# sakehl/SKA-SDP-Accelerate-gridding

Measured on AMD Instinct MI355X. Metric: Mvis/s gridded (w-proj, 4096^2 grid), higher is better.
Workload: dtype f64

## Files before the change

ska-sdp-accelerate-gridding_amd/csrc/tile_sorted.hip:

```cpp
#include "tile_common.h"

namespace gridhip {

__device__ __forceinline__ double readlane_f64(double x, int l)
{
    return __hiloint2double(__builtin_amdgcn_readlane(__double2hiint(x), l),
                            __builtin_amdgcn_readlane(__double2loint(x), l));
}

constexpr int SORTED_IM_OFF = 65528;

__device__ const int cut15[3][16] = {{0, 106, 211, 317, 422, 500, 578, 655, 733, 781, 829, 877, 926, 958, 991, 1024},
                                     {0, 108, 221, 329, 434, 513, 596, 677, 754, 800, 852, 898, 943, 969, 998, 1024},
                                     {0, 100, 202, 303, 401, 480, 562, 641, 718, 769, 824, 875, 925, 957, 992, 1024}};

struct SortedItem {
    int32_t valid, tile, grp, staged;
};

template <int S, bool DEGRID, int ABL = 0, bool AW = false, bool BT = false>
__global__ void __launch_bounds__(1024, 4) tile_grid_sorted_kernel(Geom g, const RecWord *__restrict__ recs,
                                                                const int32_t *__restrict__ bin_start,
                                                                const int32_t *__restrict__ work_start,
                                                                const double2 *__restrict__ gcf,
                                                                double2 *__restrict__ vis,
                                                                double *__restrict__ grid, int nkeys, int batch,
                                                                int32_t *__restrict__ scalars,
                                                                double2 *__restrict__ sorted_vals,
                                                                uint2 *__restrict__ sorted_mo)
{
    extern __shared__ double lds[];
    constexpr int S2 = S * S;
    constexpr int TAIL0 = S2 - ((S2 + 63) / 64 - 1) * 64;
    constexpr int EXTRA = DEGRID ? 0 : (TAIL0 > 32 && TAIL0 <= 34) ? TAIL0 - 32 : (S2 > 256 && TAIL0 <= 2) ? TAIL0 : 0;
    constexpr int S2E = S2 - EXTRA;
    constexpr int NSTEP_ALL = (S2E + 63) / 64;
    constexpr int TAIL = S2E - (NSTEP_ALL - 1) * 64;
    constexpr int MAXST = DEGRID ? 4 : 5;
    constexpr int FP = (NSTEP_ALL + MAXST - 1) / MAXST;
    constexpr int KST = (NSTEP_ALL + FP - 1) / FP;
    constexpr int REM = NSTEP_ALL % FP;
    constexpr int PBASE = NSTEP_ALL / FP;
    constexpr int NSTEP = KST;
    constexpr int LASTS = (REM == 0 ? KST : KST - 1) - 1;
    constexpr bool PAIR = !DEGRID && TAIL == 32;
    const int tid = threadIdx.x, nthr = blockDim.x;
    const int lane = tid & 63, wave = __builtin_amdgcn_readfirstlane(tid >> 6), nw = nthr >> 6;
    const int plane = g.lrows * g.ldw;
    const int IMO = BT ? g.imoff / 8 : SORTED_IM_OFF / 8;
    double *lre = lds, *lim = lds + IMO;
    int32_t *hist = reinterpret_cast<int32_t *>(lim + plane);
    const int hist_words = (nkeys + 1 + 3) & ~3;
    SortedItem *desc = reinterpret_cast<SortedItem *>(hist + hist_words);
    double2 *svals_wg = sorted_vals + (size_t)blockIdx.x * 2 * batch;
    uint2 *smo_wg = sorted_mo + (size_t)blockIdx.x * 2 * batch;
    int32_t *sorig_wg = reinterpret_cast<int32_t *>(sorted_vals) + (size_t)blockIdx.x * 2 * batch;

    constexpr bool STAGE_VALS = !DEGRID && AW;
    constexpr bool STAGE_ORIG = DEGRID && AW;
    const bool solo = nw == 1;
    const bool is_sorter = wave == nw - 1;
    if (is_sorter && !solo && !(g.dbg & 512)) __builtin_amdgcn_s_setprio(3);
    const bool is_walker = solo || !is_sorter;
    const int nwalk = solo ? 1 : nw - 1;
    const int ncell = g.lrows * g.lcols;

    if (blockIdx.x == 0 && tid == 0) {
        long long *st = reinterpret_cast<long long *>(scalars + 20);
        st[0] = (long long)__builtin_amdgcn_s_memtime();
        st[1] = (long long)__builtin_amdgcn_s_memrealtime();
    }
    long long prof[7] = {0, 0, 0, 0, 0, 0, 0}, pt = 0;
#define GH_STAMP(i_)                        \
    if ((ABL & 16) && lane == 0) {          \
        const long long now_ = clock64();   \
        prof[i_] += now_ - pt;              \
        pt = now_;                          \
    }
    if ((ABL & 16) && lane == 0) pt = clock64();

    int32_t *queue = scalars + 4;
    int turn = 0;
    int items_left = ((int)blockIdx.x >= g.npersist) ? g.budget : 0x7fffffff;
    auto prepare = [&](int slot) {
        WorkItem w;
        int grp = 0;
        bool have = false;
        if (items_left <= 0) turn = g.ngroups;
        --items_left;
        while (turn < g.ngroups) {
            grp = (blockIdx.x + turn) % g.ngroups;
            int item = 0;
            if (lane == 0) item = atomicAdd(&queue[grp], 1);
            item = __builtin_amdgcn_readfirstlane(item);
            if (find_work_at(g, bin_start, work_start, grp, item, &w)) {
                have = true;
                break;
            }
            ++turn;
        }
        if (!have) {
            if (lane == 0) desc[slot].valid = 0;
            return;
        }
        GH_STAMP(0)
        const int first_plane = (grp * g.W + g.ngroups - 1) / g.ngroups;
        const int first_slice = first_plane * g.Q * g.Q * g.P;
        double2 *svals = svals_wg + (size_t)slot * batch;
        uint2 *smo = smo_wg + (size_t)slot * batch;
        int32_t *sorig = sorig_wg + (size_t)slot * batch;
        const int b_lo = w.v_lo;
        const int cnt = min(batch, w.v_hi - b_lo);
        for (int i = lane; i <= nkeys; i += 64) hist[i] = 0;
        __builtin_amdgcn_fence(__ATOMIC_ACQ_REL, "wavefront");
        __builtin_amdgcn_wave_barrier();
        for (int r0 = lane; r0 < cnt; r0 += 8 * 64) {
            int key[8];
#pragma unroll
            for (int q = 0; q < 8; ++q) {
                bool off;
                key[q] = load_rec(recs, b_lo + min(r0 + q * 64, cnt - 1), g, &off).kslice - first_slice;
                if (AW) key[q] = (int)((unsigned)key[q] % (unsigned)nkeys);
                if (off) key[q] = -1;
            }
#pragma unroll
            for (int q = 0; q < 8; ++q)
                if (r0 + q * 64 < cnt && (unsigned)key[q] < (unsigned)nkeys) atomicAdd(&hist[key[q]], 1);
        }
        __builtin_amdgcn_fence(__ATOMIC_ACQ_REL, "wavefront");
        __builtin_amdgcn_wave_barrier();
        GH_STAMP(1)
        {
            const int per = (nkeys + 63) / 64;
            const int lo = min(lane * per, nkeys), hi = min(lo + per, nkeys);
            int sum = 0;
            for (int i = lo; i < hi; ++i) sum += hist[i];
            int incl = sum;
#pragma unroll
            for (int off = 1; off < 64; off <<= 1) {
                const int t = __shfl_up(incl, off, 64);
                if (lane >= off) incl += t;
            }
            int base = incl - sum;
            for (int i = lo; i < hi; ++i) {
                const int c = hist[i];
                hist[i] = base;
                base += c;
            }
        }
        __builtin_amdgcn_fence(__ATOMIC_ACQ_REL, "wavefront");
        __builtin_amdgcn_wave_barrier();
        GH_STAMP(2)
        int bad = 0;
        for (int r0 = lane; r0 < cnt; r0 += 8 * 64) {
            VisRec rec[8];
            double2 val[8];
            bool off[8];
#pragma unroll
            for (int q = 0; q < 8; ++q) rec[q] = load_rec(recs, b_lo + min(r0 + q * 64, cnt - 1), g, &off[q]);
            if (STAGE_VALS) {
#pragma unroll
                for (int q = 0; q < 8; ++q) val[q] = (ABL & 8) ? make_double2(1.0, (double)q) : load_nt(vis + rec[q].orig);
            }
#pragma unroll
            for (int q = 0; q < 8; ++q) {
                if (r0 + q * 64 >= cnt) break;
                int key = rec[q].kslice - first_slice;
                if (AW) key = (int)((unsigned)key % (unsigned)nkeys);
                if (off[q] || (unsigned)key >= (unsigned)nkeys) {
                    ++bad;
                    continue;
                }
                const int pos = atomicAdd(&hist[key], 1);
                if ((unsigned)pos < (unsigned)batch) {
                    smo[pos] = make_uint2(((uint32_t)key << 16) | (uint32_t)((rec[q].lxy >> 16) * g.ldw + (rec[q].lxy & 0xffff)),
                                          (uint32_t)(AW ? rec[q].kslice : rec[q].orig));
                    if (STAGE_VALS) svals[pos] = val[q];
                    if (STAGE_ORIG) sorig[pos] = rec[q].orig;
                } else
                    ++bad;
            }
        }
        if (bad) atomicAdd(&scalars[2], bad);
        __builtin_amdgcn_fence(__ATOMIC_ACQ_REL, "wavefront");
        __builtin_amdgcn_wave_barrier();
        if (lane == 0) {
            SortedItem d;
            d.valid = 1;
            d.tile = w.tile;
            d.grp = grp;
            d.staged = hist[nkeys - 1];
            desc[slot] = d;
        }
        GH_STAMP(3)
    };

    int loff[NSTEP];
    const bool tail_ok = lane < TAIL || TAIL == 64;
#pragma unroll
    for (int s = 0; s < NSTEP; ++s) {
        int t = s * 64 + lane;
        if (FP == 1 && s == NSTEP - 1 && !tail_ok) t = PAIR ? s * 64 + lane - 32 : 0;
        loff[s] = (t / S) * g.ldw + (t % S);
    }
    const int ttail = tail_ok ? LASTS * 64 + lane : PAIR ? LASTS * 64 + lane - 32 : 0;
    const int lrow = lane / S, lcol = lane - lrow * S;

    auto walk = [&](int slot, int staged, int first_slice) {
        const double2 *svals = svals_wg + (size_t)slot * batch;
        const uint2 *smo = smo_wg + (size_t)slot * batch;
        const int32_t *sorig = sorig_wg + (size_t)slot * batch;
        int seg_lo, seg_hi;
        if (nwalk == 15 && !DEGRID && !(g.dbg & 256)) {
            seg_lo = (int)(((int64_t)staged * cut15[g.dense][wave]) >> 10);
            seg_hi = (int)(((int64_t)staged * cut15[g.dense][wave + 1]) >> 10);
        } else {
            seg_lo = (int)(((int64_t)staged * wave) / nwalk);
            seg_hi = (int)(((int64_t)staged * (wave + 1)) / nwalk);
        }
        if (seg_lo >= seg_hi) return;
        auto load_list = [&](int b0, uint2 &mo, double2 &v, int32_t &o) {
            const int idx = max(min(b0 + lane, seg_hi - 1), seg_lo);
            mo = smo[idx];
            if (STAGE_VALS) v = svals[idx];
            if (STAGE_ORIG) o = sorig[idx];
        };
        auto load_value = [&](const uint2 &mo, double2 &v) {
            if (!DEGRID && !STAGE_VALS) v = (ABL & 8) ? make_double2(1.0, 2.0) : load_nt(vis + mo.y);
        };
        auto part_step0 = [&](int part) { return FP == 1 ? 0 : part * PBASE + min(part, REM); };
        auto part_nst = [&](int part) { return (FP == 1 || REM == 0 || part < REM) ? KST : KST - 1; };
        auto issue = [&](double2(&k)[NSTEP], int key, int len, int part) {
            key = min(max(key, 0), (AW ? g.nslices : nkeys) - 1);
            asm volatile("" : "+s"(key));
            const double2 *kp = gcf + (size_t)(first_slice + key) * S2 + 64 * part_step0(part);
            if (ABL & 4) {
#pragma unroll
                for (int s = 0; s < NSTEP; ++s) k[s] = make_double2((double)key, (double)(lane + s));
                return;
            }
            const int lofs = len > 0 ? lane : 0, lt = len > 0 ? ttail : 0;
            if (FP == 1) {
#pragma unroll
                for (int s = 0; s < NSTEP - 1; ++s) k[s] = kp[s * 64 + lofs];
                k[NSTEP - 1] = kp[lt];
            } else {
                const bool lastp = part == FP - 1, shortp = part_nst(part) < KST;
#pragma unroll
                for (int s = 0; s < NSTEP; ++s) {
                    int idx = s * 64 + lofs;
                    if (s == LASTS && lastp) idx = lt;
                    if (s == KST - 1 && shortp) idx = 0;
                    k[s] = kp[idx];
                }
            }
        };
        uint2 moN, moNN;
        double2 vN = make_double2(0.0, 0.0), vNN = make_double2(0.0, 0.0);
        int32_t oN = 0, oNN = 0;
        load_list(seg_lo, moN, vN, oN);
        load_list(seg_lo + 64, moNN, vNN, oNN);
        load_value(moN, vN);
        for (int b0 = seg_lo; b0 < seg_hi; b0 += 64) {
            const uint2 mo = moN;
            const double2 vB = vN;
            const int32_t oB = oN;
            moN = moNN;
            vN = vNN;
            oN = oNN;
            load_value(moN, vN);
            load_list(b0 + 128, moNN, vNN, oNN);
            const int bcnt = min(64, seg_hi - b0);
            const uint32_t mykey = AW ? mo.y : mo.x >> 16;
            const uint32_t prevkey = (uint32_t)__shfl_up((int)mykey, 1, 64);
            unsigned long long bits = __ballot(lane < bcnt && (lane == 0 || mykey != prevkey));
            double2 kx[EXTRA > 0 ? EXTRA : 1];
            if (EXTRA > 0) {
                const double2 *kp = gcf + (size_t)(first_slice + min((int)mykey, (AW ? g.nslices : nkeys) - 1)) * S2 + (S2 - EXTRA);
#pragma unroll
                for (int e = 0; e < EXTRA; ++e) kx[e] = (ABL & 4) ? make_double2(1.0, 2.0) : kp[e];
            }
            int lastKey = 0;
            int curKey = 0, curStart = 0, curLen = 0, curPart = FP - 1;
            auto advance = [&](int &key, int &start, int &len, int &part) {
                if (FP > 1 && curLen > 0 && curPart < FP - 1) {
                    ++curPart;
                    key = curKey;
                    start = curStart;
                    len = curLen;
                    part = curPart;
                    return;
                }
                if (bits == 0) {
                    key = lastKey;
                    start = 0;
                    len = 0;
                    if (FP > 1) part = FP - 1;
                    curLen = 0;
                    return;
                }
                start = (int)__builtin_ctzll(bits);
                bits &= bits - 1;
                len = (bits ? (int)__builtin_ctzll(bits) : bcnt) - start;
                key = lastKey = AW ? __builtin_amdgcn_readlane((int)mo.y, start)
                                   : (int)((uint32_t)__builtin_amdgcn_readlane((int)mo.x, start) >> 16);
                if (FP > 1) {
                    part = 0;
                    curKey = key;
                    curStart = start;
                    curLen = len;
                    curPart = 0;
                }
            };
            auto process = [&](const double2(&k)[NSTEP], int start, int len, int part) {
                int lo[NSTEP];
                const bool lastp = FP == 1 || part == FP - 1;
                const bool shortp = FP > 1 && part_nst(part) < KST;
                if (FP == 1) {
#pragma unroll
                    for (int s = 0; s < NSTEP; ++s) lo[s] = loff[s];
                } else {
                    const int st0 = part_step0(part);
#pragma unroll
                    for (int s = 0; s < NSTEP; ++s) {
                        const int tl = 64 * (st0 + s);
                        const int A = tl / S, B = tl - A * S;
                        int lr = lrow, lc = lcol;
                        if (PAIR && s == LASTS && lastp && lane >= 32) {
                            lr = (lane - 32) / S;
                            lc = (lane - 32) - lr * S;
                        }
                        const int carry = (B + lc >= S) ? g.ldw - S : 0;
                        lo[s] = (A + lr) * g.ldw + B + lc + carry;
                    }
                }
                if (!DEGRID) {
                    int i = 0;
                    if (PAIR && lastp) {
                        for (; i + 1 < len; i += 2) {
                            const int j0 = start + i, j1 = j0 + 1;
                            const int lb0 = (int)((uint32_t)__builtin_amdgcn_readlane((int)mo.x, j0) & 0xffff);
                            const int lb1 = (int)((uint32_t)__builtin_amdgcn_readlane((int)mo.x, j1) & 0xffff);
                            const double vx0 = readlane_f64(vB.x, j0), vy0 = readlane_f64(vB.y, j0);
                            const double vx1 = readlane_f64(vB.x, j1), vy1 = readlane_f64(vB.y, j1);
#pragma unroll
                            for (int s = 0; s < LASTS; ++s) {
                                double *cell = lre + (lb0 + lo[s]);
                                if (ABL & 1) continue;
                                __hip_atomic_fetch_add(cell, vx0 * k[s].x - vy0 * k[s].y, __ATOMIC_RELAXED,
                                                       __HIP_MEMORY_SCOPE_WORKGROUP);
                                __hip_atomic_fetch_add(cell + IMO, vx0 * k[s].y + vy0 * k[s].x,
                                                       __ATOMIC_RELAXED, __HIP_MEMORY_SCOPE_WORKGROUP);
                            }
#pragma unroll
                            for (int s = 0; s < LASTS; ++s) {
                                double *cell = lre + (lb1 + lo[s]);
                                if (ABL & 1) continue;
                                __hip_atomic_fetch_add(cell, vx1 * k[s].x - vy1 * k[s].y, __ATOMIC_RELAXED,
                                                       __HIP_MEMORY_SCOPE_WORKGROUP);
                                __hip_atomic_fetch_add(cell + IMO, vx1 * k[s].y + vy1 * k[s].x,
                                                       __ATOMIC_RELAXED, __HIP_MEMORY_SCOPE_WORKGROUP);
                            }
                            const double2 kl = k[LASTS];
                            double re, im;
                            int a;
                            if (lane < 32) {
                                re = vx0 * kl.x - vy0 * kl.y;
                                im = vx0 * kl.y + vy0 * kl.x;
                                a = lb0 + lo[LASTS];
                                asm volatile("" : "+v"(a));
                            } else {
                                re = vx1 * kl.x - vy1 * kl.y;
                                im = vx1 * kl.y + vy1 * kl.x;
                                a = lb1 + lo[LASTS];
                                asm volatile("" : "+v"(a));
                            }
                            if (!(ABL & 1)) {
                                __hip_atomic_fetch_add(lre + a, re, __ATOMIC_RELAXED, __HIP_MEMORY_SCOPE_WORKGROUP);
                                __hip_atomic_fetch_add(lre + a + IMO, im, __ATOMIC_RELAXED,
                                                       __HIP_MEMORY_SCOPE_WORKGROUP);
                            }
                        }
                    }
                    for (; i < len; ++i) {
                        const int j = start + i;
                        const uint32_t m = (uint32_t)__builtin_amdgcn_readlane((int)mo.x, j);
                        const int lbase = (int)(m & 0xffff);
                        const double vx = readlane_f64(vB.x, j), vy = readlane_f64(vB.y, j);
#pragma unroll
                        for (int s = 0; s < NSTEP; ++s) {
                            if (FP > 1 && s == KST - 1 && shortp) continue;
                            const double re = vx * k[s].x - vy * k[s].y;
                            const double im = vx * k[s].y + vy * k[s].x;
                            double *cell = lre + (lbase + lo[s]);
                            if (ABL & 1) {
                                if (re == 1.2345e300 || im == 1.2345e300) *cell = re;
                                continue;
                            }
                            if (TAIL == 64 || s != LASTS || !lastp || tail_ok) {
                                __hip_atomic_fetch_add(cell, re, __ATOMIC_RELAXED, __HIP_MEMORY_SCOPE_WORKGROUP);
                                __hip_atomic_fetch_add(cell + IMO, im, __ATOMIC_RELAXED,
                                                       __HIP_MEMORY_SCOPE_WORKGROUP);
                            }
                        }
                    }
                } else {
                    const double2 kz = tail_ok ? k[LASTS] : make_double2(0.0, 0.0);
                    for (int i = 0; i < len; i += 4) {
                        double sr[4], si[4];
                        int32_t oo[4];
#pragma unroll
                        for (int q = 0; q < 4; ++q) {
                            sr[q] = 0.0;
                            si[q] = 0.0;
                            oo[q] = 0;
                            if (i + q < len) {
                                const int j = start + i + q;
                                const uint32_t m = (uint32_t)__builtin_amdgcn_readlane((int)mo.x, j);
                                const int lbase = (int)(m & 0xffff);
                                oo[q] = __builtin_amdgcn_readlane(STAGE_ORIG ? (int)oB : (int)mo.y, j);
                                double gr[NSTEP], gi[NSTEP];
#pragma unroll
                                for (int s = 0; s < NSTEP; ++s) {
                                    const bool nostep = FP > 1 && s == KST - 1 && shortp;
                                    const bool idle = TAIL != 64 && s == LASTS && lastp && !tail_ok;
                                    const double *cell = lre + (lbase + ((idle || nostep) ? lo[0] : lo[s]));
                                    gr[s] = cell[0];
                                    gi[s] = cell[IMO];
                                }
#pragma unroll
                                for (int s = 0; s < NSTEP; ++s) {
                                    double2 kk = (TAIL != 64 && s == LASTS && lastp) ? kz : k[s];
                                    if (FP > 1 && s == KST - 1 && shortp) kk = make_double2(0.0, 0.0);
                                    sr[q] = fma(kk.x, gr[s], sr[q]);
                                    sr[q] = fma(-kk.y, gi[s], sr[q]);
                                    si[q] = fma(kk.x, gi[s], si[q]);
                                    si[q] = fma(kk.y, gr[s], si[q]);
                                }
                            }
                        }
                        const double rr = wave_sum4_rows(sr[0], sr[1], sr[2], sr[3]);
                        const double ri = wave_sum4_rows(si[0], si[1], si[2], si[3]);
                        const int row = lane >> 4;
                        if ((lane & 15) == 15 && i + row < len) {
                            const int32_t o = row == 0 ? oo[0] : row == 1 ? oo[1] : row == 2 ? oo[2] : oo[3];
                            if (g.P == 1 && FP == 1)
                                __builtin_nontemporal_store(dvec2_t{rr, ri}, reinterpret_cast<dvec2_t *>(vis + o));
                            else {
                                double *dst = reinterpret_cast<double *>(vis + o);
                                unsafeAtomicAdd(dst, rr);
                                unsafeAtomicAdd(dst + 1, ri);
                            }
                        }
                    }
                }
            };

            constexpr int NSETS = 3;
            double2 kS[NSETS][NSTEP];
            int keyS[NSETS], startS[NSETS], lenS[NSETS], partS[NSETS] = {0, 0, 0};
            static_assert(NSETS == 3, "initialiser of partS");
#pragma unroll
            for (int r = 0; r < NSETS - 1; ++r) {
                advance(keyS[r], startS[r], lenS[r], partS[r]);
                issue(kS[r], keyS[r], lenS[r], partS[r]);
            }
            int done = 0;
            for (;;) {
#pragma unroll
                for (int r = 0; r < NSETS; ++r) {
                    const int nx = (r + NSETS - 1) % NSETS;
                    advance(keyS[nx], startS[nx], lenS[nx], partS[nx]);
                    issue(kS[nx], keyS[nx], lenS[nx], partS[nx]);
                    asm volatile("" ::: "memory");
                    __builtin_amdgcn_sched_barrier(0);
                    process(kS[r], startS[r], lenS[r], partS[r]);
                    __builtin_amdgcn_sched_barrier(0);
                    if (FP == 1 || partS[r] == FP - 1) done += lenS[r];
                }
                if (done >= bcnt) break;
            }
            if (done > bcnt) {
#pragma unroll
                for (int r = 0; r < NSETS - 1; ++r) asm volatile("" ::"v"(kS[r][0].x), "v"(kS[r][NSTEP - 1].y));
            }
            if (EXTRA > 0 && !(ABL & 1) && lane < bcnt) {
                const int lb = (int)(mo.x & 0xffff);
#pragma unroll
                for (int e = 0; e < EXTRA; ++e) {
                    const int t = S2 - EXTRA + e;
                    double *cell = lre + (lb + (t / S) * g.ldw + (t % S));
                    __hip_atomic_fetch_add(cell, vB.x * kx[e].x - vB.y * kx[e].y, __ATOMIC_RELAXED,
                                           __HIP_MEMORY_SCOPE_WORKGROUP);
                    __hip_atomic_fetch_add(cell + IMO, vB.x * kx[e].y + vB.y * kx[e].x, __ATOMIC_RELAXED,
                                           __HIP_MEMORY_SCOPE_WORKGROUP);
                }
            }
        }
    };

    const int fl_r0 = (tid >> 1) / g.lcols, fl_c0 = (tid >> 1) - fl_r0 * g.lcols;
    const int fl_dr = (nthr >> 1) / g.lcols, fl_dc = (nthr >> 1) - fl_dr * g.lcols;

    if (is_sorter) prepare(0);
    if (!DEGRID) {
        for (int i = tid; i < plane; i += nthr) {
            lre[i] = 0.0;
            lim[i] = 0.0;
        }
    }
    __syncthreads();
    for (int cur = 0;; cur ^= 1) {
        const SortedItem d = desc[cur];
        if (!d.valid) break;
        const int first_plane = (d.grp * g.W + g.ngroups - 1) / g.ngroups;
        const int first_slice = first_plane * g.Q * g.Q * g.P;
        const int tx = d.tile % g.ntx, ty = d.tile / g.ntx;
        const int64_t ox = (int64_t)tx * g.Tx - g.offx, oy = (int64_t)ty * g.Ty - g.offy;
        if (DEGRID) {
            const double2 *gsrc = reinterpret_cast<const double2 *>(grid);
            for (int c = tid; c < ncell; c += nthr) {
                const int r_ = c / g.lcols, c_ = c - r_ * g.lcols;
                const int64_t gx = ox + c_, gy = oy + r_;
                double2 v = make_double2(0.0, 0.0);
                if (gx >= 0 && gy >= 0 && gx < g.Wd && gy < g.H) v = gsrc[gy * g.Wd + gx];
                lre[r_ * g.ldw + c_] = v.x;
                lim[r_ * g.ldw + c_] = v.y;
            }
            __syncthreads();
        }
        const long long walk_t0 = (ABL & 16) ? clock64() : 0;
        if (is_sorter && !solo) prepare(cur ^ 1);
        if (is_walker) {
            if ((ABL & 16) && wave == 0 && lane == 0) pt = clock64();
            walk(cur, d.staged, first_slice);
            if ((ABL & 16) && wave == 0) GH_STAMP(4)
        }
        if (solo) prepare(cur ^ 1);
        if ((ABL & 16) && lane == 0)
            atomicAdd(reinterpret_cast<unsigned long long *>(scalars + 32) + 8 + wave, (unsigned long long)(clock64() - walk_t0));
        __syncthreads();
        if ((ABL & 16) && wave == 0) GH_STAMP(5)
        if (DEGRID) continue;

        {
            const int comp = tid & 1;
            int r_ = fl_r0, c_ = fl_c0;
            for (int e = tid; e < 2 * ncell; e += nthr) {
                const int64_t gx = ox + c_, gy = oy + r_;
                double *cell = (comp ? lim : lre) + r_ * g.ldw + c_;
                c_ += fl_dc;
                r_ += fl_dr;
                if (c_ >= g.lcols) {
                    c_ -= g.lcols;
                    ++r_;
                }
                const double val = *cell;
                if (val == 0.0) continue;
                *cell = 0.0;
                if ((ABL & 2) || gx < 0 || gy < 0 || gx >= g.Wd || gy >= g.H) continue;
                unsafeAtomicAdd(grid + 2 * (gy * g.Wd + gx) + comp, val);
            }
        }
        __syncthreads();
        if ((ABL & 16) && wave == 0) GH_STAMP(6)
    }
    if (blockIdx.x == 0 && tid == 0) {
        long long *st = reinterpret_cast<long long *>(scalars + 20);
        st[2] = (long long)__builtin_amdgcn_s_memtime();
        st[3] = (long long)__builtin_amdgcn_s_memrealtime();
    }
    if ((ABL & 16) && lane == 0 && (wave == 0 || (is_sorter && !solo))) {
        unsigned long long *out = reinterpret_cast<unsigned long long *>(scalars + 32);
        for (int i = 0; i < 7; ++i)
            if (prof[i]) atomicAdd(&out[i], (unsigned long long)prof[i]);
    }
#undef GH_STAMP
}

bool sorted_plan(const gridhip_ctx *ctx, const Geom &g, int block, int *nkeys, int *batch, size_t *lds_bytes)
{
    if (g.gh != g.gw || g.gh < 5 || g.gh > (g.per_vis ? 16 : 32)) return false;
    const int planes = (g.W + g.ngroups - 1) / g.ngroups + 1;
    const int64_t keys = g.per_vis ? 4096 : (int64_t)planes * g.Q * g.Q * g.P;
    if (keys >= 65536) return false;
    const size_t plane = (size_t)g.lrows * g.ldw * 8;
    if (plane > (size_t)(g.imoff > 0 ? g.imoff : SORTED_IM_OFF)) return false;
    const size_t tile = (size_t)(g.imoff > 0 ? g.imoff : SORTED_IM_OFF) + plane;
    const size_t hist = (size_t)((keys + 1 + 3) & ~3) * 4;
    if (tile + hist + 128 > (size_t)ctx->max_lds) return false;
    (void)block;
    int c = ctx->opt.chunk ? (int)ctx->opt.chunk : 16384;
    c = c < 64 ? 64 : c > 16384 ? 16384 : c;
    *nkeys = (int)keys;
    *batch = c;
    *lds_bytes = tile + hist + 128;
    return true;
}

int launch_tile_grid_sorted(gridhip_ctx *ctx, const Geom &g_in, int block, size_t lds_bytes, int nkeys, int batch,
                            int64_t n, const double *gcf, const double *vis, double *grid, bool degrid)
{
    Geom g = g_in;
    Tables t = tables_of(ctx, g);
    const RecWord *recs = (const RecWord *)ctx->recs.ptr;
    if (g.chunk > batch) return fail(ctx, GRIDHIP_EINVAL, "sorted kernel: chunk %d exceeds its work-item capacity %d", g.chunk, batch);
    if (g.per_vis && g.imoff > 0) return fail(ctx, GRIDHIP_EUNSUPPORTED, "no big-tile form of the aw tile kernel");
    int per_cu = (int)((size_t)ctx->max_lds / lds_bytes);
    per_cu = per_cu < 1 ? 1 : per_cu > 4 ? 4 : per_cu;
    if (per_cu * block > 2048) per_cu = 2048 / block > 0 ? 2048 / block : 1;
    int cus = ctx->num_cu - (int)ctx->opt.reserve_cus;
    if (cus < g.ngroups) cus = g.ngroups;
    int nblk = cus * per_cu;
    nblk = ctx->opt.reserve_cus ? (nblk / g.ngroups) * g.ngroups : ((nblk + g.ngroups - 1) / g.ngroups) * g.ngroups;
    const int most = work_blocks(g, n);
    if (nblk > most) nblk = most > g.ngroups ? (most / g.ngroups) * g.ngroups : g.ngroups;
    g.npersist = nblk;
    g.budget = 0;
    if (ctx->opt.yield_cus > 0 && !ctx->opt.reserve_cus) {
        int k = (((int)ctx->opt.yield_cus + 31) / 32) * 32 * per_cu;
        k = (k / g.ngroups) * g.ngroups;
        if (k > 0 && nblk - k >= g.ngroups) {
            g.npersist = nblk - k;
            g.budget = 8;
            int extra = most - g.npersist;
            extra = extra > 2048 ? 2048 : extra;
            extra = (extra / g.ngroups) * g.ngroups;
            nblk = g.npersist + (extra > k ? extra : k);
        }
    }
    const dim3 gr(nblk), bl(block);
    const size_t nlist = (size_t)nblk * 2 * batch, nvals = g.per_vis ? nlist : 0;
    GH_CHECK(ws_reserve(ctx, ctx->sorted, nvals * 16 + nlist * 8));
    double2 *svals = (double2 *)ctx->sorted.ptr;
    uint2 *smo = (uint2 *)(svals + nvals);
    launch_clear(ctx, t.scalars + 4, 16, (g.dbg & 16) ? t.scalars + 32 : nullptr, (g.dbg & 16) ? 64 : 0);
#define GH_LAUNCH_(S_, D_, B_)                                                                                   \
    do {                                                                                                         \
        GH_CHECK(raise_lds(ctx, tile_grid_sorted_kernel<S_, D_, 0, false, B_>));                                 \
        hipLaunchKernelGGL((tile_grid_sorted_kernel<S_, D_, 0, false, B_>), gr, bl, lds_bytes, ctx->stream, g, recs, \
                           t.bin_start, t.work_start, (const double2 *)gcf, (double2 *)vis, grid, nkeys, batch, \
                           t.scalars, svals, smo);                                                               \
    } while (0)
#define GH_LAUNCH(S_, D_)                \
    do {                                 \
        if (g.imoff > 0)                 \
            GH_LAUNCH_(S_, D_, true);    \
        else                             \
            GH_LAUNCH_(S_, D_, false);   \
    } while (0)
#define GH_LAUNCH_AW_(S_, D_)                                                                                    \
    do {                                                                                                         \
        GH_CHECK(raise_lds(ctx, tile_grid_sorted_kernel<S_, D_, 0, true>));                                      \
        hipLaunchKernelGGL((tile_grid_sorted_kernel<S_, D_, 0, true>), gr, bl, lds_bytes, ctx->stream, g, recs,  \
                           t.bin_start, t.work_start, (const double2 *)gcf, (double2 *)vis, grid, nkeys, batch, \
                           t.scalars, svals, smo);                                                               \
    } while (0)
#define GH_LAUNCH_AW(S_)                 \
    do {                                 \
        if (degrid)                      \
            GH_LAUNCH_AW_(S_, true);     \
        else                             \
            GH_LAUNCH_AW_(S_, false);    \
    } while (0)
#define GH_CASE(S_)             \
    case S_:                    \
        if (g.per_vis)          \
            GH_LAUNCH_AW(S_);   \
        else if (degrid)        \
            GH_LAUNCH(S_, true); \
        else                    \
            GH_LAUNCH(S_, false); \
        break;
#define GH_BIG(S_)                                                                  \
    case S_:                                                                        \
        if (g.per_vis) return fail(ctx, GRIDHIP_EUNSUPPORTED, "aw tile kernel: support %d", g.gh); \
        if (degrid)                                                                 \
            GH_LAUNCH(S_, true);                                                    \
        else                                                                        \
            GH_LAUNCH(S_, false);                                                   \
        break;
#define GH_ABL_BT(A_)                                                                                            \
    if (g.gh == 15 && !degrid && g.imoff > 0 && g.dbg == A_) {                                                   \
        GH_CHECK(raise_lds(ctx, tile_grid_sorted_kernel<15, false, A_, false, true>));                           \
        hipLaunchKernelGGL((tile_grid_sorted_kernel<15, false, A_, false, true>), gr, bl, lds_bytes, ctx->stream, g, recs, \
                           t.bin_start, t.work_start, (const double2 *)gcf, (double2 *)vis, grid, nkeys, batch, \
                           t.scalars, svals, smo);                                                               \
        GH_CHECK_HIP(ctx, hipGetLastError());                                                                    \
        return GRIDHIP_OK;                                                                                       \
    }
#define GH_ABL(A_)                                                                                               \
    if (g.gh == 15 && !degrid && g.imoff == 0 && g.dbg == A_) {                                                  \
        GH_CHECK(raise_lds(ctx, tile_grid_sorted_kernel<15, false, A_>));                                        \
        hipLaunchKernelGGL((tile_grid_sorted_kernel<15, false, A_>), gr, bl, lds_bytes, ctx->stream, g, recs,    \
                           t.bin_start, t.work_start, (const double2 *)gcf, (double2 *)vis, grid, nkeys, batch, \
                           t.scalars, svals, smo);                                                               \
        GH_CHECK_HIP(ctx, hipGetLastError());                                                                    \
        return GRIDHIP_OK;                                                                                       \
    }
#ifdef GRIDHIP_TUNING
    GH_ABL(1) GH_ABL(2) GH_ABL(3) GH_ABL(4) GH_ABL(5) GH_ABL(7) GH_ABL(8) GH_ABL(15) GH_ABL(16) GH_ABL_BT(16)
#endif
#undef GH_ABL
#undef GH_ABL_BT
    switch (g.gh) {
        GH_CASE(5) GH_CASE(6) GH_CASE(7) GH_CASE(8) GH_CASE(9) GH_CASE(10) GH_CASE(11) GH_CASE(12) GH_CASE(13)
        GH_CASE(14) GH_CASE(15) GH_CASE(16)
        GH_BIG(17) GH_BIG(18) GH_BIG(19) GH_BIG(20) GH_BIG(21) GH_BIG(22) GH_BIG(23) GH_BIG(24) GH_BIG(25) GH_BIG(26)
        GH_BIG(27) GH_BIG(28) GH_BIG(29) GH_BIG(30) GH_BIG(31) GH_BIG(32)
        default: return fail(ctx, GRIDHIP_EUNSUPPORTED, "no sorted instantiation for support %d", g.gh);
    }
#undef GH_CASE
#undef GH_BIG
#undef GH_LAUNCH
#undef GH_LAUNCH_
#undef GH_LAUNCH_AW
#undef GH_LAUNCH_AW_
    GH_CHECK_HIP(ctx, hipGetLastError());
    return GRIDHIP_OK;
}

}
```

Baseline: 9184.

## Prefetch next tile's sorted lists and visibilities during flush, defer per-block loads

The sorted-list and visibility loads that start each walk now run earlier. For the next work item they are issued before the LDS flush to global atomics, so their latency overlaps that flush. Inside each 64-entry block, the next-block list, value and extra kernel loads are moved after the first kernel-issue step, placed with sched_barriers. This is meant to hide the startup latency of each walk and keep the block loads from stalling the first accumulation. New profiling stamps are also added under the ABL&16 flag. The cost is more live registers across the flush and a tighter instruction-scheduling constraint.

```diff
diff --git a/ska-sdp-accelerate-gridding_amd/csrc/tile_sorted.hip b/ska-sdp-accelerate-gridding_amd/csrc/tile_sorted.hip
--- a/ska-sdp-accelerate-gridding_amd/csrc/tile_sorted.hip
+++ b/ska-sdp-accelerate-gridding_amd/csrc/tile_sorted.hip
@@ -70,7 +70,7 @@
         st[0] = (long long)__builtin_amdgcn_s_memtime();
         st[1] = (long long)__builtin_amdgcn_s_memrealtime();
     }
-    long long prof[7] = {0, 0, 0, 0, 0, 0, 0}, pt = 0;
+    long long prof[9] = {0, 0, 0, 0, 0, 0, 0, 0, 0}, pt = 0;
 #define GH_STAMP(i_)                        \
     if ((ABL & 16) && lane == 0) {          \
         const long long now_ = clock64();   \
@@ -206,11 +206,22 @@
     const int ttail = tail_ok ? LASTS * 64 + lane : PAIR ? LASTS * 64 + lane - 32 : 0;
     const int lrow = lane / S, lcol = lane - lrow * S;
 
-    auto walk = [&](int slot, int staged, int first_slice) {
-        const double2 *svals = svals_wg + (size_t)slot * batch;
-        const uint2 *smo = smo_wg + (size_t)slot * batch;
-        const int32_t *sorig = sorig_wg + (size_t)slot * batch;
-        int seg_lo, seg_hi;
+    int seg_slot = 0, seg_lo = 0, seg_hi = 0;
+    uint2 moN = make_uint2(0, 0), moNN = make_uint2(0, 0);
+    double2 vN = make_double2(0.0, 0.0), vNN = make_double2(0.0, 0.0);
+    int32_t oN = 0, oNN = 0;
+    auto load_list = [&](int b0, uint2 &mo, double2 &v, int32_t &o) {
+        const int idx = min(max(min(b0 + lane, seg_hi - 1), seg_lo), batch - 1);
+        mo = (smo_wg + (size_t)seg_slot * batch)[idx];
+        if (STAGE_VALS) v = (svals_wg + (size_t)seg_slot * batch)[idx];
+        if (STAGE_ORIG) o = (sorig_wg + (size_t)seg_slot * batch)[idx];
+    };
+    auto load_value = [&](const uint2 &mo, double2 &v) {
+        if (!DEGRID && !STAGE_VALS) v = (ABL & 8) ? make_double2(1.0, 2.0) : load_nt(vis + mo.y);
+    };
+    auto open_lists = [&](int slot, int staged) {
+        const int wave = min(__builtin_amdgcn_readfirstlane(tid >> 6), nwalk - 1);
+        seg_slot = slot;
         if (nwalk == 15 && !DEGRID && !(g.dbg & 256)) {
             seg_lo = (int)(((int64_t)staged * cut15[g.dense][wave]) >> 10);
             seg_hi = (int)(((int64_t)staged * cut15[g.dense][wave + 1]) >> 10);
@@ -218,16 +229,17 @@
             seg_lo = (int)(((int64_t)staged * wave) / nwalk);
             seg_hi = (int)(((int64_t)staged * (wave + 1)) / nwalk);
         }
+        load_list(seg_lo, moN, vN, oN);
+        load_list(seg_lo + 64, moNN, vNN, oNN);
+    };
+    auto open_values = [&]() {
+        if (seg_lo < seg_hi) load_value(moN, vN);
+    };
+    auto walk = [&](int first_slice) {
         if (seg_lo >= seg_hi) return;
-        auto load_list = [&](int b0, uint2 &mo, double2 &v, int32_t &o) {
-            const int idx = max(min(b0 + lane, seg_hi - 1), seg_lo);
-            mo = smo[idx];
-            if (STAGE_VALS) v = svals[idx];
-            if (STAGE_ORIG) o = sorig[idx];
-        };
-        auto load_value = [&](const uint2 &mo, double2 &v) {
-            if (!DEGRID && !STAGE_VALS) v = (ABL & 8) ? make_double2(1.0, 2.0) : load_nt(vis + mo.y);
-        };
+        const bool stamping = (ABL & 16) && wave == 0;
+        const long long t_open = stamping ? clock64() : 0;
+        bool opened = false;
         auto part_step0 = [&](int part) { return FP == 1 ? 0 : part * PBASE + min(part, REM); };
         auto part_nst = [&](int part) { return (FP == 1 || REM == 0 || part < REM) ? KST : KST - 1; };
         auto issue = [&](double2(&k)[NSTEP], int key, int len, int part) {
@@ -255,31 +267,36 @@
                 }
             }
         };
-        uint2 moN, moNN;
-        double2 vN = make_double2(0.0, 0.0), vNN = make_double2(0.0, 0.0);
-        int32_t oN = 0, oNN = 0;
-        load_list(seg_lo, moN, vN, oN);
-        load_list(seg_lo + 64, moNN, vNN, oNN);
-        load_value(moN, vN);
         for (int b0 = seg_lo; b0 < seg_hi; b0 += 64) {
+            const long long t_top = stamping ? clock64() : 0;
+            bool first_acc = true;
             const uint2 mo = moN;
             const double2 vB = vN;
             const int32_t oB = oN;
             moN = moNN;
             vN = vNN;
             oN = oNN;
-            load_value(moN, vN);
-            load_list(b0 + 128, moNN, vNN, oNN);
             const int bcnt = min(64, seg_hi - b0);
             const uint32_t mykey = AW ? mo.y : mo.x >> 16;
             const uint32_t prevkey = (uint32_t)__shfl_up((int)mykey, 1, 64);
             unsigned long long bits = __ballot(lane < bcnt && (lane == 0 || mykey != prevkey));
             double2 kx[EXTRA > 0 ? EXTRA : 1];
-            if (EXTRA > 0) {
-                const double2 *kp = gcf + (size_t)(first_slice + min((int)mykey, (AW ? g.nslices : nkeys) - 1)) * S2 + (S2 - EXTRA);
-#pragma unroll
-                for (int e = 0; e < EXTRA; ++e) kx[e] = (ABL & 4) ? make_double2(1.0, 2.0) : kp[e];
-            }
+            auto block_loads = [&]() {
+                int bn = b0 + 128;
+                asm volatile("" : "+s"(bn));
+                if (EXTRA > 0) {
+                    int xkey = min((int)mykey, (AW ? g.nslices : nkeys) - 1);
+                    asm volatile("" : "+v"(xkey));
+                    const double2 *kp = gcf + (size_t)(first_slice + xkey) * S2 + (S2 - EXTRA);
+#pragma unroll
+                    for (int e = 0; e < EXTRA; ++e) kx[e] = (ABL & 4) ? make_double2(1.0, 2.0) : kp[e];
+                }
+                load_list(bn, moNN, vNN, oNN);
+                uint2 moV = moN;
+                asm volatile("" : "+v"(moV.y));
+                load_value(moV, vN);
+            };
+            bool top = true;
             int lastKey = 0;
             int curKey = 0, curStart = 0, curLen = 0, curPart = FP - 1;
             auto advance = [&](int &key, int &start, int &len, int &part) {
@@ -472,8 +489,24 @@
                     const int nx = (r + NSETS - 1) % NSETS;
                     advance(keyS[nx], startS[nx], lenS[nx], partS[nx]);
                     issue(kS[nx], keyS[nx], lenS[nx], partS[nx]);
+                    if (r == 0 && top) {
+                        asm volatile("" ::: "memory");
+                        __builtin_amdgcn_sched_barrier(0);
+                        block_loads();
+                        top = false;
+                    }
                     asm volatile("" ::: "memory");
                     __builtin_amdgcn_sched_barrier(0);
+                    if (stamping && first_acc) {
+                        asm volatile("" ::"v"(kS[r][0].x), "v"(vB.x));
+                        const long long now = clock64();
+                        if (lane == 0) {
+                            prof[8] += now - t_top;
+                            if (!opened) prof[7] += now - t_open;
+                        }
+                        opened = true;
+                        first_acc = false;
+                    }
                     process(kS[r], startS[r], lenS[r], partS[r]);
                     __builtin_amdgcn_sched_barrier(0);
                     if (FP == 1 || partS[r] == FP - 1) done += lenS[r];
@@ -510,6 +543,11 @@
         }
     }
     __syncthreads();
+    if (!DEGRID) {
+        const SortedItem d0 = desc[0];
+        open_lists(0, (is_walker && d0.valid) ? d0.staged : 0);
+        open_values();
+    }
     for (int cur = 0;; cur ^= 1) {
         const SortedItem d = desc[cur];
         if (!d.valid) break;
@@ -528,12 +566,14 @@
                 lim[r_ * g.ldw + c_] = v.y;
             }
             __syncthreads();
+            open_lists(cur, is_walker ? d.staged : 0);
+            open_values();
         }
         const long long walk_t0 = (ABL & 16) ? clock64() : 0;
         if (is_sorter && !solo) prepare(cur ^ 1);
         if (is_walker) {
             if ((ABL & 16) && wave == 0 && lane == 0) pt = clock64();
-            walk(cur, d.staged, first_slice);
+            walk(first_slice);
             if ((ABL & 16) && wave == 0) GH_STAMP(4)
         }
         if (solo) prepare(cur ^ 1);
@@ -543,6 +583,10 @@
         if ((ABL & 16) && wave == 0) GH_STAMP(5)
         if (DEGRID) continue;
 
+        {
+            const SortedItem dn = desc[cur ^ 1];
+            open_lists(cur ^ 1, (is_walker && dn.valid) ? dn.staged : 0);
+        }
         {
             const int comp = tid & 1;
             int r_ = fl_r0, c_ = fl_c0;
@@ -562,6 +606,7 @@
                 unsafeAtomicAdd(grid + 2 * (gy * g.Wd + gx) + comp, val);
             }
         }
+        open_values();
         __syncthreads();
         if ((ABL & 16) && wave == 0) GH_STAMP(6)
     }
@@ -574,6 +619,8 @@
         unsigned long long *out = reinterpret_cast<unsigned long long *>(scalars + 32);
         for (int i = 0; i < 7; ++i)
             if (prof[i]) atomicAdd(&out[i], (unsigned long long)prof[i]);
+        for (int i = 7; i < 9; ++i)
+            if (prof[i]) atomicAdd(&out[24 + i - 7], (unsigned long long)prof[i]);
     }
 #undef GH_STAMP
 }
```

Result: no change. 9227 (median of 6 runs) (+0.5%).
